# LilYau350/Variance-Aware-Weight

Measured on AMD Instinct MI355X. Metric: training images/sec, higher is better.
Workload: dtype bf16; 1 GPU; DiT-B/4, 4x32x32 latents, 1000 classes; Trainer.train_step: q_sample + fwd + lambda-weighted MSE + bwd + AdamW + EMA; global batch 256 = 256 per GPU; global_batch=256, per_gpu_batch=256, parallelism=dp1, weight_type=lambda, hip_graph=False

## Files before the change

### include/vaw_hip.h

```cpp
#ifndef VAW_HIP_H
#define VAW_HIP_H
#include <stdint.h>

#ifdef __cplusplus
extern "C" {
#endif

typedef enum { VAW_OK = 0, VAW_ERR_INVALID = -1, VAW_ERR_LAUNCH = -2, VAW_ERR_UNSUPPORTED = -3 } vaw_status;
typedef enum { VAW_F32 = 0, VAW_BF16 = 1,
               VAW_FP8 = 2, VAW_BF8 = 3  } vaw_dtype;
typedef void* vaw_stream;

int vaw_version(void);
const char* vaw_last_error_string(void);


int vaw_qsample_fwd(const float* x0, const float* noise, const int64_t* t, const float* tab_a, const float* tab_s,
                    int num_timesteps, float* x_t, int B, int64_t per_sample, vaw_stream stream);

int vaw_mix_rows(const float* x, const float* y, const float* ca, const float* cb, float* out, int B,
                 int64_t per_sample, vaw_stream stream);

int vaw_wmse_fwd(const float* model_out, const float* x0, const float* noise, const float* ca, const float* cb,
                 const float* w, float* mse, int B, int64_t per_sample, vaw_stream stream);
// ... 84 lines not shown
int vaw_flow_logp_prior(const float* z, double* logp, double* partials, int64_t partials_cap, int B, int64_t per_sample,
                        vaw_stream stream);


#define VAW_RESAMPLER_MAX_T 4096

int vaw_resampler_update(const int64_t* ts, const float* losses, int n, int T, int H, double* ring, int64_t* seen, int* bad,
                         vaw_stream stream);

int vaw_resampler_draw(const double* ring, const int64_t* seen, int T, int H, double uniform_prob, const double* u, int B,
                       int64_t* out_t, float* out_w, double* p, vaw_stream stream);


int vaw_row_sqnorms(const float* X, int64_t n, int D, float* out, vaw_stream stream);

int64_t vaw_pairwise_workspace_bytes(int64_t nu, int64_t nv, int k1);
int vaw_pairwise_ksmallest(const float* U, int64_t nu, const float* V, int64_t nv, int D, const float* norm_u, const float* norm_v,
                           int k1, float* out, void* ws, int64_t ws_bytes, vaw_stream stream);

int vaw_ksmallest_merge(const float* parts, int64_t n, int P, int k1, int64_t part_stride, int64_t row_stride, float* out,
                        vaw_stream stream);

int vaw_pairwise_within(const float* U, int64_t nu, const float* V, int64_t nv, int D, const float* norm_u, const float* norm_v,
                        const float* radii_u, int Ku, const float* radii_v, int Kv, uint8_t* u_in, uint8_t* v_in, vaw_stream stream);

int64_t vaw_pairwise_polysum_workspace_bytes(int64_t nu, int64_t nv, int batches);
int vaw_pairwise_polysum(const float* U, int64_t nu, const float* V, int64_t nv, int D, const int32_t* u_idx, const int32_t* v_idx, int batches,
                         double gamma, double coef0, int degree, int skip_diagonal, double* rowsum, void* ws, int64_t ws_bytes,
                         vaw_stream stream);

int64_t vaw_pairwise_count_workspace_bytes(int64_t nu, int64_t nv, int Kv);
int vaw_pairwise_count_within(const float* U, int64_t nu, const float* V, int64_t nv, int D, const float* norm_u, const float* norm_v,
                              const float* radii_v, int Kv, int32_t* u_count, uint8_t* v_in, void* ws, int64_t ws_bytes, vaw_stream stream);

int vaw_col_mean_f64(const float* X, int64_t n, int D, double* mu, vaw_stream stream);
int vaw_cov_f64(const float* X, int64_t n, int D, const double* mu, double* sigma, vaw_stream stream);

int vaw_head_logits(const float* X, int64_t n, int D, const float* Wt, int C, float* logits, int64_t ld, vaw_stream stream);
int vaw_is_rows(const float* in, int64_t n, int C, int64_t ld, int probs, double* lse, double* h, vaw_stream stream);
int vaw_is_colsums(const float* in, const double* lse, int64_t n, int C, int64_t ld, int probs, int64_t row0, int64_t split_size, double* colsum,
                   vaw_stream stream);
int vaw_is_finish(const double* h, const double* colsum, int64_t N, int C, int64_t split_size, double* scores, vaw_stream stream);


typedef struct {
    const float* bias;
    int act;
    const void* aux_in;
    void* aux_out;
    const float* gate;
    int64_t gate_ld;
    const void* resid;
    const float* rowadd;
    int rows_per_batch;
    float alpha;
    float beta;
    int out_f32;
    float* colsum_out;
    float colsum_beta;
    int resid_is_act;
    float* rowsum_a_out;
    float rowsum_a_beta;
    float* colsum_partial_out;
    int64_t* colsum_rows_out;
} vaw_epilogue;

int vaw_gemm(vaw_dtype dt, int a_kmajor, int b_kmajor, int64_t M, int64_t N, int64_t K, const void* A, int64_t lda,
             const void* B, int64_t ldb, void* C, int64_t ldc, const vaw_epilogue* epi_host, float* workspace,
             int64_t workspace_floats, vaw_stream stream);

typedef struct {
    const void* dy;
    const void* x;
    float* dw;
    int64_t M, N, ld_dy, ld_x, ld_dw;
    float alpha;
    int pad_;
    const float* scale_dy;
    const float* scale_x;
} vaw_wgrad_problem;
int64_t vaw_wgrad_grouped_desc_bytes(int n_problems);
int vaw_wgrad_grouped(vaw_dtype dt, int n_problems, const vaw_wgrad_problem* problems, int64_t K, float beta, void* desc_dev,
                      int upload, float* workspace, int64_t workspace_floats, vaw_stream stream);

int64_t vaw_fp8_quantize_workspace_floats(void);
int vaw_fp8_quantize(vaw_dtype src_dt, vaw_dtype dst_format, const void* src, int64_t R, int64_t C, int64_t ld, void* q, int64_t ldq,
                     void* qt, int64_t ldt, float* scale_out, float* workspace, int64_t workspace_floats, vaw_stream stream);
int vaw_fp8_quantize_delayed(vaw_dtype src_dt, vaw_dtype dst_format, const void* src, int64_t R, int64_t C, int64_t ld, void* q,
                             int64_t ldq, void* qt, int64_t ldt, float* state, vaw_stream stream);
int vaw_fp8_scale_update(float* states, int64_t n, vaw_stream stream);
typedef struct {
    const float* src;
    void* q;
    void* qt;
    float* state;
    int64_t R, C, ld, ldq, ldt;
} vaw_fp8_quant_job;
int64_t vaw_fp8_quantize_batched_desc_bytes(int n_jobs);
int vaw_fp8_quantize_delayed_batched(int n_jobs, const vaw_fp8_quant_job* jobs, void* desc_dev, int upload, vaw_stream stream);
int vaw_gemm_fp8(vaw_dtype a_format, int64_t M, int64_t N, int64_t K, const void* A, int64_t lda, const float* scale_a,
                 const void* B, int64_t ldb, const float* scale_b, void* C, int64_t ldc, const vaw_epilogue* epi_host,
                 float* c_fp8_state, vaw_dtype c_fp8_format, float* workspace, int64_t workspace_floats, vaw_stream stream);
int vaw_fp8_transpose(const void* q, int64_t R, int64_t C, int64_t ldq, void* qt, int64_t ldt, vaw_stream stream);

void vaw_p8_set_reserved_cus(int n);
int vaw_gemm_uses_bf16_mfma(vaw_dtype dt, int64_t M, int64_t N, int64_t K, const void* A, int64_t lda, const void* B,
                            int64_t ldb);

typedef struct {
    int tile;
    int force_generic;
    int bk;
    int pd, ws;
    int xcdsplit;
    int sm_max_m, sm_wide_m, sm_nb, sm_stages;
    int ws_loaders;
    int epi, debug;
    int p8_nt, nt_aux;
    int cus;
} vaw_gemm_knobs;
void vaw_gemm_default_knobs(vaw_gemm_knobs* out);
typedef enum {
    VAW_GV_GENERIC = 0,
    VAW_GV_T128_BK32 = 1,
    VAW_GV_T128_BK64 = 2,
    VAW_GV_RING256 = 3,
    VAW_GV_PERSISTENT = 4,
    VAW_GV_SMALL_M = 5,
    VAW_GV_PARKED_DRAIN = 6,
    VAW_GV_WARP_SPEC = 7
} vaw_gemm_variant;
typedef enum { VAW_GR_NONE = 0, VAW_GR_F32 = 1, VAW_GR_BF16 = 2, VAW_GR_F32_ROWSUM = 3 } vaw_gemm_reduce;
typedef enum { VAW_GS_NONE = 0, VAW_GS_FUSED = 1, VAW_GS_SEPARATE = 2 } vaw_gemm_rowsum_mode;
typedef enum { VAW_GC_NONE = 0, VAW_GC_FOLD = 1, VAW_GC_DEFERRED = 2, VAW_GC_SEPARATE = 3 } vaw_gemm_colsum_mode;
typedef struct {
    int variant;
    int ntw;
    int mb, nb, stages;
    int bkt;
    int epi_kind;
    int split;
    int xcd_parts;
    int grid_x, grid_y, grid_z, block;
    int64_t lds_bytes;
    int reduce;
    int rowsum_mode;
    int colsum_mode;
    int64_t colsum_rows;
    int64_t workspace_floats_used;
    int launches;
    int status;
} vaw_gemm_launch;
int vaw_gemm_plan(vaw_dtype dt, int a_kmajor, int b_kmajor, int64_t M, int64_t N, int64_t K, int64_t lda, int64_t ldb,
                  int64_t ldc, int64_t A, int64_t B, int64_t C, const vaw_epilogue* epi_host, int64_t workspace_floats,
                  const vaw_gemm_knobs* knobs, vaw_gemm_launch* out);

typedef struct {
    int epi_kind;
    int a_e5m2;
    int c_fp8, c_e5m2;
    int ntw;
    int tiles_m, tiles_n;
    int nk;
    int split;
    int grid, block;
    int64_t lds_bytes;
// ... 263 lines not shown
```

### variance-aware-weight_amd/_lib.py

```python
import ctypes as C
import os

import torch

_HERE = os.path.dirname(os.path.abspath(__file__))
LIB_PATH = os.environ.get("VAW_HIP_LIB") or os.path.join(_HERE, "libvaw_hip.so")

F32, BF16, FP8, BF8 = 0, 1, 2, 3
TORCH_DTYPE = {F32: torch.float32, BF16: torch.bfloat16}

_p, _i, _l, _f, _d = C.c_void_p, C.c_int, C.c_int64, C.c_float, C.c_double


class Epilogue(C.Structure):
    _fields_ = [("bias", _p), ("act", _i), ("aux_in", _p), ("aux_out", _p), ("gate", _p), ("gate_ld", _l),
                ("resid", _p), ("rowadd", _p), ("rows_per_batch", _i), ("alpha", _f), ("beta", _f), ("out_f32", _i),
                ("colsum_out", _p), ("colsum_beta", _f), ("resid_is_act", _i), ("rowsum_a_out", _p), ("rowsum_a_beta", _f),
                ("colsum_partial_out", _p), ("colsum_rows_out", C.POINTER(C.c_int64))]


class AttnDesc(C.Structure):
    _fields_ = [("B", _i), ("H", _i), ("T", _i), ("hd", _i), ("q_sb", _l), ("q_sh", _l), ("q_st", _l), ("q_sd", _l),
                ("o_sb", _l), ("o_sh", _l), ("o_st", _l), ("o_sd", _l), ("scale", _f)]

# ... 181 lines not shown
    "vaw_cast_colsum_bf16": [_p, _l, _p, _l, _l, _l, _p, _f, _p],
    "vaw_row_sqnorms": [_p, _l, _i, _p, _p],
    "vaw_pairwise_ksmallest": [_p, _l, _p, _l, _i, _p, _p, _i, _p, _p, _l, _p],
    "vaw_ksmallest_merge": [_p, _l, _i, _i, _l, _l, _p, _p],
    "vaw_pairwise_within": [_p, _l, _p, _l, _i, _p, _p, _p, _i, _p, _i, _p, _p, _p],
    "vaw_pairwise_polysum": [_p, _l, _p, _l, _i, _p, _p, _i, _d, _d, _i, _i, _p, _p, _l, _p],
    "vaw_pairwise_count_within": [_p, _l, _p, _l, _i, _p, _p, _p, _i, _p, _p, _p, _l, _p],
    "vaw_col_mean_f64": [_p, _l, _i, _p, _p],
    "vaw_cov_f64": [_p, _l, _i, _p, _p, _p],
    "vaw_head_logits": [_p, _l, _i, _p, _i, _p, _l, _p],
    "vaw_is_rows": [_p, _l, _i, _l, _i, _p, _p, _p],
    "vaw_is_colsums": [_p, _p, _l, _i, _l, _i, _l, _l, _p, _p],
    "vaw_is_finish": [_p, _p, _l, _i, _l, _p, _p],
}

_lib = None


class VawError(RuntimeError):
    pass


def lib():
    global _lib
    if _lib is None:
        if not os.path.exists(LIB_PATH):
            raise VawError(f"{LIB_PATH} not found: build it with `python -c 'import __graft_entry__ as g; g.build()'` "
                           "(there is no CPU fallback for the HIP path)")
        L = C.CDLL(LIB_PATH)
        for name, args in _PROTOS.items():
            if not hasattr(L, name) and os.environ.get("VAW_HIP_LIB"):
                continue
            fn = getattr(L, name)
            fn.argtypes = args
            fn.restype = _i
        L.vaw_version.restype = _i
        L.vaw_last_error_string.restype = C.c_char_p
        L.vaw_colsum_workspace_floats.argtypes = [_l, _l]
        L.vaw_colsum_workspace_floats.restype = _l
        L.vaw_row_bwd_workspace_floats.argtypes = [_i, _i, _i]
        L.vaw_row_bwd_workspace_floats.restype = _l
        L.vaw_conv3x3_wgrad_small_workspace_floats.argtypes = [_i, _i, _i, _i, _i]
        L.vaw_conv3x3_wgrad_small_workspace_floats.restype = _l
        L.vaw_groupnorm_workspace_floats.argtypes = [_i, _i, _i]
        L.vaw_groupnorm_workspace_floats.restype = _l
        if hasattr(L, "vaw_dropout_bits_words"):
            L.vaw_dropout_bits_words.argtypes = [_l]
            L.vaw_dropout_bits_words.restype = _l
        L.vaw_wgrad_grouped_desc_bytes.argtypes = [_i]
        L.vaw_wgrad_grouped_desc_bytes.restype = _l
        L.vaw_reduce_rows_batched_desc_bytes.argtypes = [_i]
        L.vaw_reduce_rows_batched_desc_bytes.restype = _l
        L.vaw_fp8_quantize_batched_desc_bytes.argtypes = [_i]
        L.vaw_fp8_quantize_batched_desc_bytes.restype = _l
        L.vaw_fp8_quantize_workspace_floats.argtypes = []
        L.vaw_fp8_quantize_workspace_floats.restype = _l
        if hasattr(L, "vaw_pairwise_workspace_bytes"):
            L.vaw_pairwise_workspace_bytes.argtypes = [_l, _l, _i]
            L.vaw_pairwise_workspace_bytes.restype = _l
        if hasattr(L, "vaw_pairwise_polysum_workspace_bytes"):
            L.vaw_pairwise_polysum_workspace_bytes.argtypes = [_l, _l, _i]
            L.vaw_pairwise_polysum_workspace_bytes.restype = _l
            L.vaw_pairwise_count_workspace_bytes.argtypes = [_l, _l, _i]
            L.vaw_pairwise_count_workspace_bytes.restype = _l
        if hasattr(L, "vaw_rk_partial_count"):
            L.vaw_rk_partial_count.argtypes = [_i, _l]
            L.vaw_rk_partial_count.restype = _l
        L.vaw_sumsq_workspace_floats.argtypes = []
        L.vaw_sumsq_workspace_floats.restype = _l
        L.vaw_debug_force_rowwise_attention.argtypes = [_i]
        L.vaw_debug_force_rowwise_attention.restype = None
        L.vaw_debug_force_generic_gemm.argtypes = [_i]
        L.vaw_debug_force_generic_gemm.restype = None
        L.vaw_debug_gemm_tile.argtypes = [_i]
        L.vaw_debug_gemm_tile.restype = None
        if hasattr(L, "vaw_gemm_default_knobs"):
            L.vaw_gemm_default_knobs.argtypes = [C.POINTER(GemmKnobs)]
            L.vaw_gemm_default_knobs.restype = None
        if hasattr(L, "vaw_debug_gn_flat"):
            L.vaw_debug_gn_flat.argtypes = [_i]
            L.vaw_debug_gn_flat.restype = None
        L.vaw_p8_set_reserved_cus.argtypes = [_i]
        L.vaw_p8_set_reserved_cus.restype = None
        L.vaw_debug_cu_hog.argtypes = [_i, _i, _p]
        L.vaw_debug_cu_hog.restype = _i
        _lib = L
    return _lib


def exported_symbols():
    return sorted(list(_PROTOS) + ["vaw_version", "vaw_last_error_string", "vaw_colsum_workspace_floats",
                                   "vaw_sumsq_workspace_floats", "vaw_groupnorm_workspace_floats", "vaw_wgrad_grouped_desc_bytes",
                                   "vaw_conv3x3_wgrad_small_workspace_floats", "vaw_row_bwd_workspace_floats",
                                   "vaw_fp8_quantize_workspace_floats", "vaw_p8_set_reserved_cus", "vaw_reduce_rows_batched_desc_bytes", "vaw_fp8_quantize_batched_desc_bytes",
                                   "vaw_gemm_default_knobs", "vaw_dropout_bits_words", "vaw_pairwise_workspace_bytes", "vaw_rk_partial_count",
                                   "vaw_pairwise_polysum_workspace_bytes", "vaw_pairwise_count_workspace_bytes"])


STEP_FUSED = os.environ.get("VAW_STEP_FUSED", "1") != "0"
ROWS_FWD_FUSED = os.environ.get("VAW_ROWS_FWD_FUSED", "1") != "0"


def check(rc, what):
    if rc != 0:
        raise VawError(f"{what} failed ({rc}): {lib().vaw_last_error_string().decode()}")


def stream_ptr():
    return torch.cuda.current_stream().cuda_stream


def ptr(t):
    return 0 if t is None else t.data_ptr()


def need_cuda(*tensors):
    for t in tensors:
        if t is not None and not t.is_cuda:
            raise VawError("vaw_amd runs on the GPU only: got a CPU tensor (no CPU fallback exists by design)")
```

### variance-aware-weight_amd/csrc/gemm_p8.hip

```cpp
#include "gemm_p8_kernel.h"
#include "gemm_plan.h"
static_assert(P8Cfg<3>::lds_bytes == vaw_lds_p8(3) && P8Cfg<4>::lds_bytes == vaw_lds_p8(4), "gemm_plan.h: LDS size of the persistent kernel");

void p8_launch_fwd(const P8Launch& L, const EpiDev& e, hipStream_t s);
void p8_launch_dgrad(const P8Launch& L, const EpiDev& e, hipStream_t s);
void p8_launch_wgrad(const P8Launch& L, const EpiDev& e, hipStream_t s);
void p8_launch_tn(const P8Launch& L, const EpiDev& e, hipStream_t s);

static int g_p8_reserved = 0;
extern "C" void vaw_p8_set_reserved_cus(int n) { g_p8_reserved = n > 0 ? n : 0; }
static int p8_num_cus() {
    static int n = 0, env_r = 0;
    if (!n) {
        int dev = 0;
        hipDeviceProp_t prop;
        if (hipGetDevice(&dev) == hipSuccess && hipGetDeviceProperties(&prop, dev) == hipSuccess) n = prop.multiProcessorCount;
        if (n <= 0) n = 256;
        const char* v = getenv("VAW_P8_RESERVE_CUS");
        env_r = v ? atoi(v) : 0;
    }
    const int r = env_r > g_p8_reserved ? env_r : g_p8_reserved;
    return (r > 0 && r < n - 8) ? n - r : n;
}

int vaw_p8_cus_available() { return p8_num_cus(); }

static double p8_cost(int64_t M, int64_t N, int ntw, int split, int cus) {
    const int bn = 64 * ntw;
    const int64_t items = ((M + 255) / 256) * ((N + bn - 1) / bn) * split;
    const int64_t rounds = (items + cus - 1) / cus;
    return (double)rounds * (ntw == 4 ? 1.0 : 0.85) / split;
}

P8Plan vaw_p8_plan(int64_t M, int64_t N, int64_t K, bool plain_f32, bool want_colsum, int64_t ws_floats, int force, int cus) {
    P8Plan pl{false, 4, 1, 0};
    if (force == 0) return pl;
    const int nk = (int)(K / 64);
    double best = 1e30;
    for (int ntw = 4; ntw >= 3; --ntw) {
        if (force == 2 && ntw != 4) continue;
        if (force == 3 && ntw != 3) continue;
        const int bn = 64 * ntw;
        const int64_t tiles = ((M + 255) / 256) * ((N + bn - 1) / bn);
        if (ntw == 3 && force != 3) {
            const int64_t pad4 = ((N + 255) / 256) * 256, pad3 = ((N + 191) / 192) * 192;
            if (pad3 > pad4) continue;
        }
        int smax = 1;
        if (plain_f32 && !want_colsum && ws_floats > 0) {
            int64_t s = nk / 4;
            if (s > ws_floats / (M * N)) s = ws_floats / (M * N);
            if (s > 64) s = 64;
            if (s > cus / tiles) s = cus / tiles;
            smax = s < 1 ? 1 : (int)s;
        }
        for (int s = 1; s <= smax; ++s) {
            const int per = (nk + s - 1) / s;
            if ((nk + per - 1) / per != s) continue;
            double c = p8_cost(M, N, ntw, s, cus) * nk;
            if (s > 1) c += 3.0;
            if (c < best - 1e-9) { best = c; pl.ntw = ntw; pl.split = s; }
        }
    }
    const int bn = 64 * pl.ntw;
    const int64_t items = ((M + 255) / 256) * ((N + bn - 1) / bn) * pl.split;
    pl.grid = (int)(items < cus ? items : cus);
    pl.use = force > 0 || (items >= cus / 2 && nk / pl.split >= 4 && M >= 256 && N >= 128);
    return pl;
}

void vaw_p8_launch(const P8Plan& pl, int epi, int a_kmajor, int b_kmajor, int64_t M, int64_t N, int64_t K, const bf16_t* a, int64_t lda,
                   const bf16_t* b, int64_t ldb, const EpiDev& e, hipStream_t s) {
    const int bn = 64 * pl.ntw;
    const int tiles_m = (int)((M + 255) / 256), tiles_n = (int)((N + bn - 1) / bn), nk = (int)(K / 64);
    static int team_pct = -1;
    if (team_pct < 0) { const char* v = getenv("VAW_P8_TEAM_PCT"); team_pct = v ? atoi(v) : 0; }
    const int64_t items = (int64_t)tiles_m * tiles_n * pl.split;
    const int nk_item = (nk + pl.split - 1) / pl.split;
    const int team_delay = (team_pct > 0 && items >= 2 * pl.grid) ? (int)(nk_item * 160LL * pl.ntw / 4 * team_pct / 100) : 0;
    P8Launch L{a, b, lda, ldb, nk, tiles_m, tiles_n, pl.split, pl.grid, pl.ntw, epi, team_delay};
    if (a_kmajor && b_kmajor) p8_launch_fwd(L, e, s);
    else if (a_kmajor && !b_kmajor) p8_launch_dgrad(L, e, s);
    else if (!a_kmajor && !b_kmajor) p8_launch_wgrad(L, e, s);
    else p8_launch_tn(L, e, s);
}

#include <vector>

void vaw_p8_group_fp8(int ntw, bool a_e5m2, int nk, int grid, const EpiDev& e, const P8Prob* probs_dev, const P8Group& grp, hipStream_t s);

extern "C" int64_t vaw_wgrad_grouped_desc_bytes(int n_problems) { return (int64_t)n_problems * (int64_t)sizeof(P8Prob); }

extern "C" int vaw_wgrad_grouped(vaw_dtype dt, int n_problems, const vaw_wgrad_problem* problems, int64_t K, float beta,
                                 void* desc_dev, int upload, float* workspace, int64_t workspace_floats, vaw_stream stream) {
    VAW_CHECK_ARG(dt == VAW_BF16 || dt == VAW_FP8 || dt == VAW_BF8, "wgrad_grouped: bf16 or fp8 operands (the f32 parity mode runs vaw_gemm per layer)");
    const bool f8 = dt == VAW_FP8 || dt == VAW_BF8;
    const int kt = f8 ? 128 : 64;
    VAW_CHECK_ARG(n_problems > 0 && problems && desc_dev && K > 0 && K % kt == 0, "wgrad_grouped: bad arguments (K %% %d)", kt);
    bool all192 = true, any_not256 = false;
    for (int i = 0; i < n_problems; ++i) {
        const vaw_wgrad_problem& q = problems[i];
        VAW_CHECK_ARG(q.dy && q.x && q.dw && q.M >= 16 && q.N >= 16 && q.M % 8 == 0 && q.N % 8 == 0, "wgrad_grouped: problem %d: M, N", i);
        if (f8) VAW_CHECK_ARG(q.ld_dy >= K && q.ld_x >= K && q.ld_dw >= q.N && q.ld_dy % 16 == 0 && q.ld_x % 16 == 0 && q.ld_dw % 4 == 0,
                              "wgrad_grouped: problem %d: leading dimensions (fp8: dy^T [M][K], x^T [N][K])", i);
        else VAW_CHECK_ARG(q.ld_dy >= q.M && q.ld_x >= q.N && q.ld_dw >= q.N && q.ld_dy % 8 == 0 && q.ld_x % 8 == 0 && q.ld_dw % 4 == 0,
                           "wgrad_grouped: problem %d: leading dimensions", i);
        VAW_CHECK_ARG((((uintptr_t)q.dy | (uintptr_t)q.x | (uintptr_t)q.dw) & 15) == 0, "wgrad_grouped: problem %d: alignment", i);
        VAW_CHECK_ARG(q.M < (1 << 30) && q.N < (1 << 30), "wgrad_grouped: problem %d too large", i);
        all192 = all192 && q.N % 192 == 0;
        any_not256 = any_not256 || q.N % 256 != 0;
    }
    const int ntw = (all192 && any_not256) ? 3 : 4, bn = 64 * ntw;
    static thread_local std::vector<P8Prob> host;
    host.resize(n_problems);
    int64_t t_total = 0;
    for (int i = 0; i < n_problems; ++i) {
        const vaw_wgrad_problem& q = problems[i];
        P8Prob& h = host[i];
        h.a = (const bf16_t*)q.dy; h.b = (const bf16_t*)q.x; h.c = q.dw;
        h.lda = q.ld_dy; h.ldb = q.ld_x; h.ldc = q.ld_dw;
        h.M = (int)q.M; h.N = (int)q.N;
        h.alpha = q.alpha != 0.f ? q.alpha : 1.f;
        h.pad_ = 0;
        h.scale_a = f8 ? q.scale_dy : nullptr;
        h.scale_b = f8 ? q.scale_x : nullptr;
        h.tiles_n = (int)((q.N + bn - 1) / bn);
        h.tile0 = (int)t_total;
        t_total += ((q.M + 255) / 256) * h.tiles_n;
        VAW_CHECK_ARG(t_total < (1 << 30), "wgrad_grouped: too many tiles");
    }
    hipStream_t s = (hipStream_t)stream;
    if (upload) {
        const hipError_t rc = vaw_upload_table(desc_dev, host.data(), sizeof(P8Prob) * n_problems, s);
        VAW_CHECK_ARG(rc == hipSuccess, "wgrad_grouped: descriptor upload failed: %s", hipGetErrorString(rc));
    }
    const int cus = p8_num_cus(), nk = (int)(K / kt);
    P8Group grp{};
    grp.n_prob = n_problems;
    grp.t_full = (int)(t_total / cus) * cus;
    grp.t_rem = (int)(t_total - grp.t_full);
    grp.n_split = 1;
    grp.slab = workspace;
    if (grp.t_rem > 0) {
        int64_t sp = cus / grp.t_rem;
        if (sp > nk / 4) sp = nk / 4;
        const int64_t per_split = (int64_t)grp.t_rem * 256 * bn;
        if (workspace_floats <= 0 || !workspace) sp = 0;
        else if (sp > workspace_floats / per_split) sp = workspace_floats / per_split;
        if (sp < 2) {
            grp.t_full = (int)t_total;
            grp.t_rem = 0;
        } else {
            const int per = (nk + (int)sp - 1) / (int)sp;
            grp.n_split = (nk + per - 1) / per;
        }
    }
    const int64_t items = grp.t_full + (int64_t)grp.t_rem * grp.n_split;
    const int grid = (int)(items < cus ? items : cus);
    EpiDev e{};
    e.alpha = 1.f;
    e.beta = beta;
    e.out_f32 = 1;
    e.rpb = 1;
    e.nt_off = 1;
    {
        static int dbg = -1;
        if (dbg < 0) { const char* v = getenv("VAW_GEMM_DEBUG"); dbg = v ? atoi(v) : 0; }
        e.debug = dbg;
    }
    if (f8) vaw_p8_group_fp8(ntw, dt == VAW_BF8, nk, grid, e, (const P8Prob*)desc_dev, grp, s);
    else if (ntw == 4) p8_launch_group<4>(nk, grid, e, (const P8Prob*)desc_dev, grp, s);
    else p8_launch_group<3>(nk, grid, e, (const P8Prob*)desc_dev, grp, s);
    if (grp.t_rem > 0) {
        if (ntw == 4) p8_group_fixup_kernel<256><<<grp.t_rem * 8, 256, 0, s>>>((const P8Prob*)desc_dev, grp, beta);
        else p8_group_fixup_kernel<192><<<grp.t_rem * 8, 256, 0, s>>>((const P8Prob*)desc_dev, grp, beta);
    }
    VAW_CHECK_LAUNCH("wgrad_grouped");
    return VAW_OK;
}
```

### variance-aware-weight_amd/ops.py

```python
import ctypes as C
import math

import numpy as np
import torch

from . import _lib as L
from ._lib import BF16, F32, AttnDesc, Epilogue, check, need_cuda, ptr, stream_ptr


def dt_of(t):
    if t.dtype == torch.float32:
        return F32
    if t.dtype == torch.bfloat16:
        return BF16
    raise L.VawError(f"unsupported activation dtype {t.dtype}")


def _f32c(*ts):
    for t in ts:
        if t is not None and (t.dtype != torch.float32 or not t.is_contiguous()):
            raise L.VawError(f"expected a contiguous float32 tensor, got {t.dtype} contiguous={t.is_contiguous()}")


def qsample(x0, noise, t, tab_a, tab_s):
# ... 612 lines not shown

def q_scratch(n, device, pool=0):
    t = _q_scratch.get((device, pool))
    if t is None or t.numel() < n:
        t = _q_scratch[(device, pool)] = torch.empty(n, device=device, dtype=torch.uint8)
    return t


def gemm_fp8(M, N, K, A, lda, scale_a, B, ldb, scale_b, Cp, ldc, *, a_format=L.FP8, bias=None, act=0, aux_in=None, aux_out=None,
             gate=None, gate_ld=0, resid=None, rows_per_batch=0, alpha=1.0, out_f32=False, colsum_out=None, colsum_beta=0.0,
             out_fp8=None, colsum_partial=None):
    e = Epilogue(bias or None, act, aux_in or None, aux_out or None, gate or None, gate_ld, resid or None, None, rows_per_batch,
                 alpha, 0.0, 1 if out_f32 else 0, colsum_out or None, colsum_beta, 0, None, 0.0)
    if colsum_partial is not None:
        colsum_partial.rows.value = colsum_partial.buf.shape[0]
        e.colsum_partial_out, e.colsum_rows_out = colsum_partial.buf.data_ptr(), C.pointer(colsum_partial.rows)
    tr = gemm_trace
    if tr is not None:
        e0, e1 = tr.events()
        e0.record()
    ws_ptr, ws_n = 0, 0
    if colsum_out:
        ws = scratch_f32(torch.device("cuda", torch.cuda.current_device()), 0)
        ws_ptr, ws_n = ws.data_ptr(), ws.numel()
    check(L.lib().vaw_gemm_fp8(a_format, M, N, K, A, lda, scale_a, B, ldb, scale_b, Cp, ldc, C.byref(e),
                               out_fp8.state.data_ptr() if out_fp8 is not None else None, out_fp8.fmt if out_fp8 is not None else 0,
                               ws_ptr, ws_n, stream_ptr()), "vaw_gemm_fp8")
    if tr is not None:
        e1.record()
        nb = M * K + N * K + M * N * ((4 if out_f32 else 1 if out_fp8 is not None else 2) + (2 if aux_out else 0) + (2 if aux_in else 0) +
                                      (4 if resid else 0))
        tr.add(2, True, a_format == L.FP8, M, N, K, e0, e1, float(nb))


def gemm_fp8_plan(M, N, K, A, lda, scale_a, B, ldb, scale_b, Cp, ldc, *, a_format=L.FP8, workspace=16, workspace_floats=0, cus=0,
                  colsum_partial_rows=None, out_fp8_state=0, out_fp8_format=L.FP8, check_status=True, **epi):
    e = Epilogue(epi.get("bias") or None, epi.get("act", 0), epi.get("aux_in") or None, epi.get("aux_out") or None, epi.get("gate") or None,
                 epi.get("gate_ld", 0), epi.get("resid") or None, epi.get("rowadd") or None, epi.get("rows_per_batch", 0),
                 epi.get("alpha", 1.0), epi.get("beta", 0.0), 1 if epi.get("out_f32") else 0, epi.get("colsum_out") or None,
                 epi.get("colsum_beta", 0.0), 1 if epi.get("resid_is_act") else 0, epi.get("rowsum_a_out") or None,
                 epi.get("rowsum_a_beta", 0.0))
    rows = C.c_int64(colsum_partial_rows or 0)
    if colsum_partial_rows is not None:
        e.colsum_partial_out, e.colsum_rows_out = epi.get("colsum_partial_out", 16), C.pointer(rows)
    p = L.GemmFp8Launch()
    rc = L.lib().vaw_gemm_fp8_plan(a_format, M, N, K, A, lda, scale_a, B, ldb, scale_b, Cp, ldc, C.byref(e), out_fp8_state, out_fp8_format,
                                   workspace if workspace_floats > 0 else 0, workspace_floats, cus, C.byref(p))
    if check_status:
        check(rc, "vaw_gemm_fp8_plan")
    return p


class WgradProblem(C.Structure):
    _fields_ = [("dy", C.c_void_p), ("x", C.c_void_p), ("dw", C.c_void_p), ("M", C.c_int64), ("N", C.c_int64),
                ("ld_dy", C.c_int64), ("ld_x", C.c_int64), ("ld_dw", C.c_int64), ("alpha", C.c_float), ("pad_", C.c_int),
                ("scale_dy", C.c_void_p), ("scale_x", C.c_void_p)]


class WgradGroup:

    def __init__(self, problems, K, device):
        self.n, self.K, self.device = len(problems), int(K), device
        self.table = (WgradProblem * self.n)(*[WgradProblem(*p) for p in problems])
        self.flop = sum(2.0 * p[3] * p[4] * K for p in problems)
        self.desc = torch.empty(L.lib().vaw_wgrad_grouped_desc_bytes(self.n), device=device, dtype=torch.uint8)
        self.uploaded = False

    def launch(self, dt, beta):
        ws = scratch_f32(self.device, 0)
        tr = gemm_trace
        if tr is not None:
            e0, e1 = tr.events()
            e0.record()
        check(L.lib().vaw_wgrad_grouped(dt, self.n, C.cast(self.table, C.c_void_p), self.K, float(beta), self.desc.data_ptr(),
                                        0 if self.uploaded else 1, ws.data_ptr(), ws.numel(), stream_ptr()), "vaw_wgrad_grouped")
        self.uploaded = True
        if tr is not None:
            e1.record()
            es = 1 if dt in (L.FP8, L.BF8) else 2
            tr.add_flop(2 if dt in (L.FP8, L.BF8) else 1, False, False, self.flop, e0, e1,
                        float(sum(es * (p.M + p.N) * self.K + 4 * p.M * p.N * (2 if beta else 1) for p in self.table)))


def beta_or_plain(bias, act, aux_out, gate, resid, rowadd):
    return not (bias or act or aux_out or gate or resid or rowadd)


def conv3x3(dt, mode, act, act2, w, out, B, H, W, Ci, Co, *, bias=None, resid=None, resid_is_act=True, beta=0.0,
            colsum_out=None, colsum_beta=0.0, rowsum_a_out=None, rowsum_a_beta=0.0):
    e = Epilogue(bias or None, 0, None, None, None, 0, resid or None, None, 0, 1.0, beta, 1 if mode == 2 else 0,
                 colsum_out or None, colsum_beta, 1 if resid_is_act else 0, rowsum_a_out or None, rowsum_a_beta)
    ws = scratch_f32(torch.device("cuda", torch.cuda.current_device()), 0)
    tr = gemm_trace
    if tr is not None:
        e0, e1 = tr.events()
        e0.record()
    rc = L.lib().vaw_conv3x3(dt, mode, act, act2 or None, w, out, B, H, W, Ci, Co, C.byref(e), ws.data_ptr(), ws.numel(), stream_ptr())
    if rc == -3:
        if dt == L.BF16:
            key = ("conv3x3", ("fwd", "dgrad", "wgrad")[mode], B, H, W, Ci, Co)
            fallbacks[key] = fallbacks.get(key, 0) + 1
            if fallbacks[key] == 1:
                import warnings
                warnings.warn(f"vaw_amd: conv3x3 {key[1]} [B={B}, {H}x{W}, Ci={Ci}, Co={Co}] is not covered by the implicit-GEMM kernels "
                              "(channel counts off the 64 / 8 grid?): falling back to im2col + GEMM; counts in vaw_amd.ops.fallbacks",
                              RuntimeWarning, stacklevel=3)
        return False
    check(rc, "vaw_conv3x3")
    if tr is not None:
        e1.record()
        M = B * H * W
        nb = 2 * M * (Ci + Co) + (2 if mode != 2 else 4 * (2 if beta else 1)) * 9 * Ci * Co + ((2 * M * Co) if (mode == 0 and resid) else 0)
        tr.add(1, mode != 2, mode == 0, *((M, Co, 9 * Ci) if mode == 0 else (M, Ci, 9 * Co) if mode == 1 else (Co, 9 * Ci, M)), e0, e1, float(nb), tag=f"conv{H}x{W}")
    return True


def conv3x3_plan(dt, mode, act, act2, w, out, B, H, W, Ci, Co, *, workspace=16, workspace_floats=0, knobs=None, cus=0, check_status=True,
                 **epi):
    e = Epilogue(epi.get("bias") or None, epi.get("act", 0), None, epi.get("aux_out") or None, epi.get("gate") or None, epi.get("gate_ld", 0),
                 epi.get("resid") or None, epi.get("rowadd") or None, 0, 1.0, epi.get("beta", 0.0),
                 1 if (mode == 2 or epi.get("out_f32")) else 0, epi.get("colsum_out") or None, epi.get("colsum_beta", 0.0),
                 1 if epi.get("resid_is_act", True) else 0, epi.get("rowsum_a_out") or None, epi.get("rowsum_a_beta", 0.0))
    p = L.Conv3x3Launch()
    rc = L.lib().vaw_conv3x3_plan(dt, mode, act or 0, act2 or 0, w or 0, out or 0, B, H, W, Ci, Co, C.byref(e),
                                  workspace if workspace_floats > 0 else 0, workspace_floats, C.byref(knobs) if knobs is not None else None,
                                  cus, C.byref(p))
    if check_status:
        check(rc, "vaw_conv3x3_plan")
    return p


fallbacks = {}


class GemmTrace:

    def __init__(self):
        self.rows = []

    def events(self):
        return torch.cuda.Event(enable_timing=True), torch.cuda.Event(enable_timing=True)

    def add(self, mfma, ak, bk, M, N, K, e0, e1, nbytes=0.0, tag="gemm"):
        self.rows.append((mfma, ak, bk, 2.0 * M * N * K, e0, e1, nbytes, (tag, int(M), int(N), int(K))))

    def add_flop(self, mfma, ak, bk, flop, e0, e1, nbytes=0.0):
        self.rows.append((mfma, ak, bk, flop, e0, e1, nbytes, None))

    @staticmethod
    def _name(mfma, ak, bk):
        return ("fp8_mfma" if mfma == 2 else "bf16_mfma" if mfma else "generic_f32mfma") + ("/fwd" if ak and bk else "/dgrad" if ak else "/wgrad")

    def by_shape(self):
        acc = {}
        for mfma, ak, bk, flop, e0, e1, nbytes, shape in self.rows:
            d = acc.setdefault((self._name(mfma, ak, bk), shape), [0, 0.0, 0.0])
            d[0] += 1
            d[1] += e0.elapsed_time(e1)
            d[2] += flop
        return sorted(((k[0], k[1], v[0], v[1], v[2]) for k, v in acc.items()), key=lambda r: -r[3])

    def summarize(self):
        out = {}
        for mfma, ak, bk, flop, e0, e1, nbytes, _shape in self.rows:
            name = self._name(mfma, ak, bk)
            d = out.setdefault(name, {"launches": 0, "flop": 0.0, "ms": 0.0, "bytes": 0.0})
# ... 481 lines not shown
```

Before: 21390 images/sec.

## Add hand-scheduled persistent bf16 wgrad grouped GEMM kernel with interleaved DMA and MFMA

```diff
diff --git a/include/vaw_hip.h b/include/vaw_hip.h
--- a/include/vaw_hip.h
+++ b/include/vaw_hip.h
@@ -190,6 +190,7 @@
 int64_t vaw_wgrad_grouped_desc_bytes(int n_problems);
 int vaw_wgrad_grouped(vaw_dtype dt, int n_problems, const vaw_wgrad_problem* problems, int64_t K, float beta, void* desc_dev,
                       int upload, float* workspace, int64_t workspace_floats, vaw_stream stream);
+void vaw_debug_wgrad_engine(int mode);
 
 int64_t vaw_fp8_quantize_workspace_floats(void);
 int vaw_fp8_quantize(vaw_dtype src_dt, vaw_dtype dst_format, const void* src, int64_t R, int64_t C, int64_t ld, void* q, int64_t ldq,
diff --git a/variance-aware-weight_amd/_lib.py b/variance-aware-weight_amd/_lib.py
--- a/variance-aware-weight_amd/_lib.py
+++ b/variance-aware-weight_amd/_lib.py
@@ -287,6 +287,9 @@
             L.vaw_debug_gn_flat.restype = None
         L.vaw_p8_set_reserved_cus.argtypes = [_i]
         L.vaw_p8_set_reserved_cus.restype = None
+        if hasattr(L, "vaw_debug_wgrad_engine"):
+            L.vaw_debug_wgrad_engine.argtypes = [_i]
+            L.vaw_debug_wgrad_engine.restype = None
         L.vaw_debug_cu_hog.argtypes = [_i, _i, _p]
         L.vaw_debug_cu_hog.restype = _i
         _lib = L
@@ -297,7 +300,7 @@
     return sorted(list(_PROTOS) + ["vaw_version", "vaw_last_error_string", "vaw_colsum_workspace_floats",
                                    "vaw_sumsq_workspace_floats", "vaw_groupnorm_workspace_floats", "vaw_wgrad_grouped_desc_bytes",
                                    "vaw_conv3x3_wgrad_small_workspace_floats", "vaw_row_bwd_workspace_floats",
-                                   "vaw_fp8_quantize_workspace_floats", "vaw_p8_set_reserved_cus", "vaw_reduce_rows_batched_desc_bytes", "vaw_fp8_quantize_batched_desc_bytes",
+                                   "vaw_fp8_quantize_workspace_floats", "vaw_p8_set_reserved_cus", "vaw_debug_wgrad_engine", "vaw_reduce_rows_batched_desc_bytes", "vaw_fp8_quantize_batched_desc_bytes",
                                    "vaw_gemm_default_knobs", "vaw_dropout_bits_words", "vaw_pairwise_workspace_bytes", "vaw_rk_partial_count",
                                    "vaw_pairwise_polysum_workspace_bytes", "vaw_pairwise_count_workspace_bytes"])
 
diff --git a/variance-aware-weight_amd/csrc/gemm_g4.hip b/variance-aware-weight_amd/csrc/gemm_g4.hip
--- /dev/null
+++ b/variance-aware-weight_amd/csrc/gemm_g4.hip
@@ -0,0 +1,5 @@
+#include "gemm_g4_kernel.h"
+
+void vaw_g4_launch_group(int nk, int grid, const EpiDev& e, const P8Prob* probs_dev, const P8Group& grp, hipStream_t s) {
+    g4_launch_group(nk, grid, e, probs_dev, grp, s);
+}
diff --git a/variance-aware-weight_amd/csrc/gemm_g4_kernel.h b/variance-aware-weight_amd/csrc/gemm_g4_kernel.h
--- /dev/null
+++ b/variance-aware-weight_amd/csrc/gemm_g4_kernel.h
@@ -0,0 +1,278 @@
+#pragma once
+#include "gemm_p8_kernel.h"
+
+#define G4_STAGE (8 * P8_PART)
+#define G4_EPI_BYTES (4 * 4096)
+#define G4_LDS_BYTES (2 * G4_STAGE + G4_EPI_BYTES)
+static_assert(G4_STAGE == P8Cfg<4>::stage_bytes, "the stage layout of gemm_p8_kernel");
+static_assert(G4_LDS_BYTES <= 160 * 1024, "LDS of one CU");
+static_assert(7 * P8_PART + 4096 + 512 < 65536, "fragment reads address a whole stage through the 16-bit DS offset");
+
+template <int OFF>
+__device__ __forceinline__ bf16x8 g4_frag(unsigned addr) {
+    bf16x4 lo, hi;
+    asm volatile("ds_read_b64_tr_b16 %0, %2 offset:%3\n\tds_read_b64_tr_b16 %1, %2 offset:%4"
+                 : "=&v"(lo), "=&v"(hi)
+                 : "v"(addr), "i"(OFF), "i"(OFF + 512)
+                 : "memory");
+    return bf16x8{lo[0], lo[1], lo[2], lo[3], hi[0], hi[1], hi[2], hi[3]};
+}
+
+#define G4_SB() __builtin_amdgcn_sched_barrier(0)
+#define G4_IC(v) std::integral_constant<int, (v)>{}
+
+__global__ void __launch_bounds__(256) __attribute__((amdgpu_waves_per_eu(1, 1)))
+gemm_g4_kernel(int nk_total, EpiDev e, const P8Prob* __restrict__ probs, P8Group grp) {
+    constexpr int BN = 256;
+    extern __shared__ __attribute__((aligned(16))) char smem[];
+    const int lane = threadIdx.x & 63;
+    const int wid = __builtin_amdgcn_readfirstlane(threadIdx.x >> 6);
+    const int wr = wid >> 1, wc = wid & 1;
+    const int G = gridDim.x;
+    const int n_items = grp.t_full + grp.t_rem * grp.n_split;
+    int it_cur;
+    {
+        const int b = blockIdx.x, x = b & 7, q = G >> 3, r = G & 7;
+        it_cur = (x < r ? x * (q + 1) : r * (q + 1) + (x - r) * q) + (b >> 3);
+    }
+    if (it_cur >= n_items) return;
+    const int nk_per = (nk_total + grp.n_split - 1) / grp.n_split;
+    auto decode = [&](int it) __attribute__((always_inline)) {
+        P8Item t;
+        int g;
+        if (it < grp.t_full) { g = it; t.split = -1; t.rem = 0; t.kt0 = 0; t.nk = nk_total; }
+        else {
+            const int j = it - grp.t_full;
+            t.split = j / grp.t_rem;
+            t.rem = j - t.split * grp.t_rem;
+            g = grp.t_full + t.rem;
+            t.kt0 = t.split * nk_per;
+            t.nk = t.kt0 + nk_per <= nk_total ? nk_per : nk_total - t.kt0;
+        }
+        int pi = 0;
+        while (pi + 1 < grp.n_prob && probs[pi + 1].tile0 <= g) ++pi;
+        const P8Prob& pr = probs[pi];
+        const int tile = g - pr.tile0, tm = tile / pr.tiles_n;
+        t.prob = pi; t.tm = tm;
+        t.a = pr.a; t.b = pr.b; t.lda = pr.lda; t.ldb = pr.ldb; t.M = pr.M; t.N = pr.N;
+        t.m0 = (int64_t)tm * P8_BM;
+        t.n0 = (int64_t)(tile - tm * pr.tiles_n) * BN;
+        return t;
+    };
+
+    int iss_item = it_cur, iss_kt = 0, iss_nk = 0, iss_stage = 0;
+    bool iss_done = false;
+    __amdgpu_buffer_rsrc_t rs_a = epi_rsrc(probs), rs_b = epi_rsrc(probs);
+    unsigned so_a = 0, so_b = 0, step_a = 0, step_b = 0;
+    u32x4_t off_a = {0, 0, 0, 0}, off_b = {0, 0, 0, 0};
+    auto iss_open = [&]() __attribute__((always_inline)) {
+        const P8Item t = decode(iss_item);
+        int lane = threadIdx.x & 63;
+        asm volatile("" : "+v"(lane));
+        iss_nk = t.nk;
+        iss_kt = 0;
+        const int mvalid = t.M - t.m0 < P8_BM ? (int)(t.M - t.m0) : P8_BM;
+        const int nvalid = t.N - t.n0 < BN ? (int)(t.N - t.n0) : BN;
+        step_a = (unsigned)(64 * t.lda * 2);
+        step_b = (unsigned)(64 * t.ldb * 2);
+        so_a = so_b = 0;
+        rs_a = epi_rsrc((const char*)t.a + (t.m0 + t.kt0 * 64 * t.lda) * 2);
+        rs_b = epi_rsrc((const char*)t.b + (t.n0 + t.kt0 * 64 * t.ldb) * 2);
+        off_a = u32x4_t{p8_src_off<false>(true, 0, wid, lane, t.lda, mvalid), p8_src_off<false>(true, 1, wid, lane, t.lda, mvalid),
+                        p8_src_off<false>(true, 2, wid, lane, t.lda, mvalid), p8_src_off<false>(true, 3, wid, lane, t.lda, mvalid)};
+        off_b = u32x4_t{p8_src_off<false>(false, 0, wid, lane, t.ldb, nvalid), p8_src_off<false>(false, 1, wid, lane, t.ldb, nvalid),
+                        p8_src_off<false>(false, 2, wid, lane, t.ldb, nvalid), p8_src_off<false>(false, 3, wid, lane, t.ldb, nvalid)};
+    };
+    auto iss_close = [&]() __attribute__((always_inline)) {
+        off_a = off_b = u32x4_t{EPI_OOB, EPI_OOB, EPI_OOB, EPI_OOB};
+    };
+    auto iss_piece = [&](auto cc, auto subc) __attribute__((always_inline)) {
+        constexpr int c = decltype(cc)::value, sub = decltype(subc)::value;
+        char* dst = smem + iss_stage * G4_STAGE + (4 * sub + wid) * 1024;
+        if constexpr (c < 4) p8_dma16(rs_b, dst + 4 * P8_PART + c * P8_PART, off_b[c], __builtin_amdgcn_readfirstlane(so_b + sub * (step_b >> 1)));
+        else p8_dma16(rs_a, dst + (c - 4) * P8_PART, off_a[c - 4], __builtin_amdgcn_readfirstlane(so_a + sub * (step_a >> 1)));
+    };
+    auto iss_advance = [&]() __attribute__((always_inline)) {
+        iss_stage ^= 1;
+        if (iss_done) return;
+        so_a += step_a;
+        so_b += step_b;
+        if (++iss_kt == iss_nk) {
+            iss_item += G;
+            if (iss_item >= n_items) { iss_done = true; iss_close(); }
+            else iss_open();
+        }
+    };
+#define G4_PIECES(SUB)                                                                                                       \
+    do {                                                                                                                     \
+        iss_piece(G4_IC(0), G4_IC(SUB)); iss_piece(G4_IC(1), G4_IC(SUB)); iss_piece(G4_IC(2), G4_IC(SUB)); iss_piece(G4_IC(3), G4_IC(SUB)); \
+        iss_piece(G4_IC(4), G4_IC(SUB)); iss_piece(G4_IC(5), G4_IC(SUB)); iss_piece(G4_IC(6), G4_IC(SUB)); iss_piece(G4_IC(7), G4_IC(SUB)); \
+    } while (0)
+
+    unsigned rA[2], rB[4];
+    {
+        const int li = lane & 15, q = li >> 2, p = li & 3;
+        const int kb0 = 8 * (lane >> 4) + q, swz = p8_mn_swz(kb0);
+        const unsigned lane_off = (unsigned)(uintptr_t)(lds_ptr_t)smem + kb0 * 128 + ((p >> 1) << 4) + 8 * (p & 1);
+#pragma unroll
+        for (int t = 0; t < 2; ++t) rA[t] = lane_off + (((4 * wr + 2 * t) ^ swz) << 4);
+#pragma unroll
+        for (int k = 0; k < 4; ++k) rB[k] = lane_off + 4 * P8_PART + 2 * wc * P8_PART + (((2 * k) ^ swz) << 4);
+    }
+    int rd_delta = G4_STAGE;
+    bf16x8 fa[2][8], fb[2][8];
+    auto read_frag = [&](auto nxc, auto fc) __attribute__((always_inline)) {
+        constexpr int nx = decltype(nxc)::value, f = decltype(fc)::value;
+        if constexpr (f < 8) fb[nx][f] = g4_frag<(f >> 2) * P8_PART + nx * 4096>(rB[f & 3]);
+        else fa[nx][f - 8] = g4_frag<((f - 8) >> 1) * P8_PART + nx * 4096>(rA[(f - 8) & 1]);
+    };
+
+    iss_open();
+    G4_PIECES(0);
+    G4_PIECES(1);
+    iss_advance();
+    G4_PIECES(0);
+    asm volatile("s_waitcnt vmcnt(8)" ::: "memory");
+    __builtin_amdgcn_s_barrier();
+    G4_SB();
+    read_frag(G4_IC(0), G4_IC(0)); read_frag(G4_IC(0), G4_IC(1)); read_frag(G4_IC(0), G4_IC(2)); read_frag(G4_IC(0), G4_IC(3));
+    read_frag(G4_IC(0), G4_IC(4)); read_frag(G4_IC(0), G4_IC(5)); read_frag(G4_IC(0), G4_IC(6)); read_frag(G4_IC(0), G4_IC(7));
+    read_frag(G4_IC(0), G4_IC(8)); read_frag(G4_IC(0), G4_IC(9)); read_frag(G4_IC(0), G4_IC(10)); read_frag(G4_IC(0), G4_IC(11));
+    read_frag(G4_IC(0), G4_IC(12)); read_frag(G4_IC(0), G4_IC(13)); read_frag(G4_IC(0), G4_IC(14)); read_frag(G4_IC(0), G4_IC(15));
+    G4_SB();
+
+    for (; it_cur < n_items; it_cur += G) {
+        const P8Item item = decode(it_cur);
+        const int split = item.split, nk = item.nk;
+        const int64_t m0 = item.m0, n0 = item.n0;
+        f32x4 acc[8][8];
+#pragma unroll
+        for (int i = 0; i < 8; ++i)
+#pragma unroll
+            for (int u = 0; u < 8; ++u) acc[i][u] = f32x4{0, 0, 0, 0};
+        auto row = [&](auto sc, auto ic) __attribute__((always_inline)) {
+            constexpr int s = decltype(sc)::value, i = decltype(ic)::value, nx = s ^ 1;
+            if constexpr (i == 0) asm volatile("s_waitcnt lgkmcnt(14)" ::: "memory");
+            else asm volatile("s_waitcnt lgkmcnt(15)" ::: "memory");
+            G4_SB();
+#define G4_MMA(u) acc[i][u] = __builtin_amdgcn_mfma_f32_16x16x32_bf16(fb[s][u], fa[s][i], acc[i][u], 0, 0, 0)
+            G4_MMA(0);
+            G4_SB();
+            read_frag(G4_IC(nx), G4_IC(2 * i));
+            G4_SB();
+            G4_MMA(1);
+            G4_MMA(2);
+            G4_SB();
+            read_frag(G4_IC(nx), G4_IC(2 * i + 1));
+            G4_SB();
+            G4_MMA(3);
+            G4_MMA(4);
+            G4_SB();
+            iss_piece(G4_IC(i), G4_IC(nx));
+            G4_SB();
+            G4_MMA(5);
+            G4_MMA(6);
+            G4_MMA(7);
+#undef G4_MMA
+            G4_SB();
+        };
+#define G4_HALF(S)                                                                                                           \
+    do {                                                                                                                     \
+        row(G4_IC(S), G4_IC(0)); row(G4_IC(S), G4_IC(1)); row(G4_IC(S), G4_IC(2)); row(G4_IC(S), G4_IC(3));                  \
+        row(G4_IC(S), G4_IC(4)); row(G4_IC(S), G4_IC(5)); row(G4_IC(S), G4_IC(6)); row(G4_IC(S), G4_IC(7));                  \
+    } while (0)
+        for (int kt = 0; kt < nk; ++kt) {
+            G4_HALF(0);
+            iss_advance();
+            asm volatile("s_waitcnt vmcnt(8)" ::: "memory");
+            __builtin_amdgcn_s_barrier();
+            G4_SB();
+#pragma unroll
+            for (int t = 0; t < 2; ++t) rA[t] += rd_delta;
+#pragma unroll
+            for (int k = 0; k < 4; ++k) rB[k] += rd_delta;
+            rd_delta = -rd_delta;
+            G4_HALF(1);
+            asm volatile("s_waitcnt vmcnt(8)" ::: "memory");
+            __builtin_amdgcn_s_barrier();
+            G4_SB();
+        }
+#undef G4_HALF
+        asm volatile("s_waitcnt lgkmcnt(0)\n\ts_nop 15" ::: "memory");
+        G4_SB();
+
+        const P8Prob& pr = probs[item.prob];
+        EpiDev ei{};
+        ei.beta = e.beta; ei.nt_off = 1; ei.out_f32 = 1; ei.rpb = 1;
+        ei.C = pr.c; ei.ldc = pr.ldc; ei.M = pr.M; ei.N = pr.N; ei.alpha = pr.alpha;
+        char* ep = smem + 2 * G4_STAGE + wid * 4096;
+        int lane_e = lane;
+        asm volatile("" : "+v"(lane_e));
+        const int wr_row = lane_e & 15, wr_g = lane_e >> 4;
+        const int rd_row = lane_e >> 3, rd_c8 = lane_e & 7;
+        const unsigned ep_base = (unsigned)(uintptr_t)(lds_ptr_t)ep;
+        const unsigned ep_w = ep_base + wr_row * 256 + ((wr_g ^ (wr_row & 3)) << 4);
+        unsigned ep_r[2];
+#pragma unroll
+        for (int pass = 0; pass < 2; ++pass) {
+            const int rr = pass * 8 + rd_row;
+            ep_r[pass] = ep_base + rr * 256 + (((2 * rd_c8) ^ rr) << 4);
+        }
+        const int64_t m_last = ei.M - 1;
+        const int64_t tile_off = m0 * ei.ldc + n0;
+        const bool to_slab = split >= 0;
+        const __amdgpu_buffer_rsrc_t rs_c =
+            to_slab ? epi_rsrc(grp.slab + ((int64_t)split * grp.t_rem + item.rem) * (P8_BM * BN)) : epi_rsrc((const float*)ei.C + tile_off);
+        const int64_t mrow0 = m0 + wr * 128 + rd_row;
+        const f32x4 b0 = {0, 0, 0, 0}, b1 = {0, 0, 0, 0};
+        const EpiOps no_ops{};
+        float qmax = 0.f;
+#pragma unroll
+        for (int hh = 0; hh < 2; ++hh) {
+            const int wn0 = wc * 128 + 64 * hh;
+            const int64_t n = n0 + wn0 + 8 * rd_c8;
+            const bool col_ok = n < ei.N;
+            const int64_t n_ld = col_ok ? n : n0;
+            const int loc_col = wn0 + 8 * rd_c8;
+#pragma unroll
+            for (int i = 0; i < 8; ++i) {
+#pragma unroll
+                for (int u = 0; u < 4; ++u)
+                    asm volatile("ds_write_b128 %0, %1" ::"v"(ep_w + (unsigned)(((4 * u) ^ (wr_row & 12)) << 4)), "a"(acc[i][4 * hh + u]) : "memory");
+#pragma unroll
+                for (int pass = 0; pass < 2; ++pass) {
+                    const int k = 2 * i + pass;
+                    const int64_t m = mrow0 + 8 * k;
+                    f32x4 v0, v1;
+                    asm volatile("ds_read_b128 %0, %2\n\tds_read_b128 %1, %3\n\ts_waitcnt lgkmcnt(0)"
+                                 : "=&v"(v0), "=&v"(v1)
+                                 : "v"(ep_r[pass]), "v"(ep_r[pass] ^ 16u)
+                                 : "memory");
+                    G4_SB();
+                    const bool ok = col_ok && m <= m_last;
+                    const int loc = ok ? (int)((m - m0) * ei.ldc) + loc_col : -1;
+                    if (to_slab) {
+                        const unsigned bo = ok ? 4u * (unsigned)((m - m0) * BN + loc_col) : EPI_OOB;
+                        buf_store16(rs_c, bo, v0, false);
+                        buf_store16(rs_c, ok ? bo + 16u : EPI_OOB, v1, false);
+                    } else {
+                        const int64_t mc = m <= m_last ? m : m_last;
+                        epi_apply8<P8_WGRAD>(ei, rs_c, rs_c, loc, (const float*)ei.C + mc * ei.ldc + n_ld, v0, v1, b0, b1, no_ops, qmax);
+                    }
+                    G4_SB();
+                }
+            }
+        }
+    }
+    asm volatile("s_waitcnt vmcnt(0) lgkmcnt(0)" ::: "memory");
+#undef G4_PIECES
+}
+
+static void g4_launch_group(int nk, int grid, const EpiDev& e, const P8Prob* probs_dev, const P8Group& grp, hipStream_t s) {
+    static bool attr_done = false;
+    if (!attr_done) {
+        (void)hipFuncSetAttribute((const void*)gemm_g4_kernel, hipFuncAttributeMaxDynamicSharedMemorySize, G4_LDS_BYTES);
+        attr_done = true;
+    }
+    gemm_g4_kernel<<<grid, 256, G4_LDS_BYTES, s>>>(nk, e, probs_dev, grp);
+}
diff --git a/variance-aware-weight_amd/csrc/gemm_p8.hip b/variance-aware-weight_amd/csrc/gemm_p8.hip
--- a/variance-aware-weight_amd/csrc/gemm_p8.hip
+++ b/variance-aware-weight_amd/csrc/gemm_p8.hip
@@ -88,6 +88,19 @@
 #include <vector>
 
 void vaw_p8_group_fp8(int ntw, bool a_e5m2, int nk, int grid, const EpiDev& e, const P8Prob* probs_dev, const P8Group& grp, hipStream_t s);
+void vaw_g4_launch_group(int nk, int grid, const EpiDev& e, const P8Prob* probs_dev, const P8Group& grp, hipStream_t s);
+
+#define G4_BY_SHAPE 1
+static int g_wgrad_engine = -2;
+static int wgrad_engine() {
+    if (g_wgrad_engine == -2) {
+        const char* v = getenv("VAW_WGRAD_ENGINE");
+        const int m = v ? atoi(v) : -1;
+        g_wgrad_engine = (m == 0 || m == 1) ? m : -1;
+    }
+    return g_wgrad_engine;
+}
+extern "C" void vaw_debug_wgrad_engine(int mode) { g_wgrad_engine = (mode == 0 || mode == 1) ? mode : -1; }
 
 extern "C" int64_t vaw_wgrad_grouped_desc_bytes(int n_problems) { return (int64_t)n_problems * (int64_t)sizeof(P8Prob); }
 
@@ -169,8 +182,11 @@
         e.debug = dbg;
     }
     if (f8) vaw_p8_group_fp8(ntw, dt == VAW_BF8, nk, grid, e, (const P8Prob*)desc_dev, grp, s);
-    else if (ntw == 4) p8_launch_group<4>(nk, grid, e, (const P8Prob*)desc_dev, grp, s);
-    else p8_launch_group<3>(nk, grid, e, (const P8Prob*)desc_dev, grp, s);
+    else if (ntw == 4) {
+        const int eng = wgrad_engine();
+        if (eng == 1 || (eng < 0 && G4_BY_SHAPE)) vaw_g4_launch_group(nk, grid, e, (const P8Prob*)desc_dev, grp, s);
+        else p8_launch_group<4>(nk, grid, e, (const P8Prob*)desc_dev, grp, s);
+    } else p8_launch_group<3>(nk, grid, e, (const P8Prob*)desc_dev, grp, s);
     if (grp.t_rem > 0) {
         if (ntw == 4) p8_group_fixup_kernel<256><<<grp.t_rem * 8, 256, 0, s>>>((const P8Prob*)desc_dev, grp, beta);
         else p8_group_fixup_kernel<192><<<grp.t_rem * 8, 256, 0, s>>>((const P8Prob*)desc_dev, grp, beta);
diff --git a/variance-aware-weight_amd/ops.py b/variance-aware-weight_amd/ops.py
--- a/variance-aware-weight_amd/ops.py
+++ b/variance-aware-weight_amd/ops.py
@@ -718,6 +718,10 @@
                         float(sum(es * (p.M + p.N) * self.K + 4 * p.M * p.N * (2 if beta else 1) for p in self.table)))
 
 
+def wgrad_engine(mode):
+    L.lib().vaw_debug_wgrad_engine(int(mode))
+
+
 def beta_or_plain(bias, act, aux_out, gate, resid, rowadd):
     return not (bias or act or aux_out or gate or resid or rowadd)
 
```

New measurement: 21870 images/sec, median of 6. 2.2% higher.
